# Dicklesworthstone/frankensearch

Hardware: AMD Instinct MI355X
Metric: queries/sec + p50 phase-1 latency, 10M×384 f16 corpus, 1/2/4/8 MI355X (higher is better)
Workload: dtype f16 x f32 -> f32 (every emitted score, in the reference's operation order); candidate filter i8 x i8 -> i32

## Files before the change

frankensearch_amd/csrc/kernels.hpp:

```cpp
#pragma once

#include <hip/hip_runtime.h>
#include <stddef.h>
#include <stdint.h>

namespace fsgpu {

typedef unsigned long long u64;

struct ScanArgs {
    const void* slab;
    const u64* live;
    const u64* allow;
    const float* queries;
    u64* partial;
    uint32_t nrows;
    uint32_t dim;
    uint32_t k;
    uint32_t row_base;
    int32_t hreduce;
    uint32_t row_stride;
};

struct MergeArgs {
// ... 153 lines not shown
                                 hipStream_t stream);
hipError_t launch_prepare_queries_i8(const float* q, uint32_t nq, uint32_t nq_pad, uint32_t dim, void* qi8, float* delta,
                                     hipStream_t stream, int bits = 8);
hipError_t launch_prepare_queries_i8_filter(const float* q, uint32_t nq, uint32_t nq_pad, uint32_t dim, uint32_t q_stride,
                                            const unsigned int* slab_max_bits, const unsigned int* slab_stats, void* qi8,
                                            float* delta, hipStream_t stream, float* unit_out = nullptr, double extra_coeff = 0.0);

constexpr uint32_t kMfmaMaxSlots = 32;
constexpr uint32_t kMfmaSpillCountStride = 16;
constexpr uint32_t kWideSlots = 32;
bool scan_mfma_supported(int dim);
bool scan_wide_supported(int dim, int elem_bytes);
bool scan_wide_group_maxima_supported(int dim, int query_tiles);
int scan_wide_max_query_tiles(int dim, int elem_bytes);
hipError_t launch_scan_wide(const MfmaScanArgs& args, int query_tiles, int grid, hipStream_t stream, int* occupancy);
bool scan_wide_flat_priority();
void note_main_pass_kernel(const char* name);
const char* last_main_pass_kernel();
int scan_mfma_waves_per_block(int shape);
int scan_mfma_rows_per_tile(int shape);
int scan_mfma_query_tiles(int shape);
int scan_mfma_max_slots(int shape);
bool scan_mfma_shape_built(int shape);
int scan_mfma_planner_shape(int requested, int elem_bytes);
hipError_t launch_scan_mfma(const MfmaScanArgs& args, int shape, int grid, hipStream_t stream, int* occupancy);
hipError_t launch_max_row_norm(const void* slab, uint32_t nrows, uint32_t dim, uint32_t row_stride_bytes, unsigned int* out_bits,
                               hipStream_t stream);
hipError_t launch_max_row_norm_f32(const float* rows, uint32_t nrows, uint32_t dim, unsigned int* out_bits, hipStream_t stream);
hipError_t launch_prepare_queries(const float* q, uint32_t nq, uint32_t nq_pad, uint32_t dim, uint32_t q_stride,
                                  const unsigned int* max_norm_bits, void* qh, float* delta, hipStream_t stream);
// ... 322 lines not shown
```

frankensearch_amd/csrc/mfma_wide.hip:

```cpp
#include <atomic>
#include <cstdlib>
#include <string>
#include <vector>
#include <type_traits>

#include "scan_common.hpp"

namespace fsgpu {

using namespace scan_detail;

typedef float f32x4 __attribute__((ext_vector_type(4)));
typedef int i32x4 __attribute__((ext_vector_type(4)));

namespace {

__device__ __forceinline__ void glds16(const void* gsrc, uint32_t lds_dst) {
    unsigned keep;
    asm volatile(
        "s_mov_b32 %0, m0\n\t"
        "s_mov_b32 m0, %2\n\t"
        "s_nop 0\n\t"
        "global_load_lds_dwordx4 %1, off\n\t"
        "s_mov_b32 m0, %0"
// ... 39 lines not shown

__device__ __forceinline__ int ceil_threshold(float t) {
    if (!(t <= 33554432.0f)) return 1 << 25;
    if (t < -33554432.0f) return -(1 << 25);
    return (int)ceilf(t);
}

__device__ __forceinline__ bool wave_any(bool x) { return __ballot(x) != 0; }

template <int N>
__device__ __forceinline__ void wait_vmcnt() {
    static_assert(N >= 0 && N < 64, "vmcnt is a 6-bit field");
    asm volatile("s_waitcnt vmcnt(%0)" ::"n"(N) : "memory");
}

[[maybe_unused]] __device__ __forceinline__ void flag_post(uint32_t lds_addr, int lane) {
    asm volatile("" ::: "memory");
    if (lane == 0) {
        const uint32_t one = 1;
        asm volatile("ds_add_u32 %0, %1" ::"v"(lds_addr), "v"(one) : "memory");
    }
}
[[maybe_unused]] __device__ __forceinline__ void flag_wait(uint32_t lds_addr, uint32_t target) {
    for (;;) {
        uint32_t v;
        asm volatile("ds_read_b32 %0, %1\n\ts_waitcnt lgkmcnt(0)" : "=v"(v) : "v"(lds_addr) : "memory");
        if ((uint32_t)__builtin_amdgcn_readfirstlane(v) >= target) break;
        __builtin_amdgcn_s_sleep(1);
    }
    asm volatile("" ::: "memory");
}

}

constexpr int kOptNegTau = 2, kOptSaddr = 4, kOptSplit = 8, kOptBig = 16, kOptFlags = 32, kOptFlat = 64;

constexpr int wide_level(int h, int H) { return 3 - (h * 4) / H; }

constexpr int wide_chunk_ksteps(int KS, int QT) {
    return KS == 12 ? (QT >= 3 ? 2 : 3) : KS == 6 ? (QT >= 5 ? 1 : 3) : KS == 4 ? (QT >= 7 ? 1 : 2) : (KS >= 2 ? KS / 2 : 1);
}
constexpr bool wide_room(int ROWB, int QT) {
    const int KS = ROWB / 64;
    return QT * KS * 4 + 4 * wide_chunk_ksteps(KS, QT) * 4 + 8 * QT <= 190;
}
constexpr bool wide_split_ok(int ROWB, int EB, int QT, int OPT, int DBG) {
    const int KS = ROWB / 64;
    return (OPT & kOptSplit) != 0 && (OPT & kOptNegTau) != 0 && EB == 1 && wide_room(ROWB, QT) && ROWB < 512 && QT >= 2 && DBG != 1 &&
           QT * KS * 4 + 2 * KS * 4 + 9 * QT <= 200;
}
// ... 48 lines not shown
    r[2] = wi;
    r[3] = (unsigned long long)which | ((unsigned long long)(uintptr_t)p << 8);
    r[4] = sv;
    r[5] = vv;
    r[6] = sv2;
    r[7] = vv2;
}
#endif

template <int ROWB, int EB, int QT, int NSLOT, int OPT, int DBG, int WPBT, int NQB>
__device__ __forceinline__ void scan_wide_body(MfmaScanArgs args, const int q0_wave) {
    using acc_t = std::conditional_t<EB == 2, f32x4, i32x4>;
    constexpr int WPB = WPBT, NT = WPB * 64;
    constexpr int KS = ROWB / 64;
    constexpr bool BIG = wide_big_ok(ROWB, EB, QT, NSLOT, OPT, DBG);
    constexpr bool FLAGS = BIG && (OPT & kOptFlags) != 0;
    constexpr int TR = BIG ? 128 : ROWB >= 512 ? 32 : 64;
    constexpr int RS = TR / 16;
    constexpr int NI = RS * KS;
    constexpr int PW = NI / WPB;
    static_assert(NI % WPB == 0 && PW >= 1, "a tile's DMA instructions divide evenly over the 8 waves");
    static_assert(RS % 2 == 0, "sub-tiles are consumed in pairs");
    constexpr int CK = wide_chunk_ksteps(KS, QT);
    constexpr int NCH = KS / CK;
    constexpr int NC = (RS / 2) * NCH;
    static_assert(KS % CK == 0 && NC % 2 == 0, "an even number of chunks per tile: the register double buffer starts every tile in the same phase");
    static_assert(NSLOT >= 3, "tile n is consumed while n+1 .. n+NSLOT-2 are in flight and n-1's slot is being refilled");
    constexpr bool ROOM = wide_room(ROWB, QT);
    constexpr bool NEGTAU = (OPT & kOptNegTau) != 0 && EB == 1 && ROOM;
    constexpr bool SADDR = (OPT & kOptSaddr) != 0 && ROOM;
    constexpr bool SPLIT = wide_split_ok(ROWB, EB, QT, OPT, DBG);
    constexpr bool LEVEL = SPLIT && (OPT & kOptFlat) == 0;
    constexpr bool GMAX = DBG == 7 && SPLIT && EB == 1;
    constexpr bool SK = DBG >= 16 && DBG < 32;
    constexpr bool SK_NO_DMA = DBG == 2 || (SK && (DBG & 1)), SK_NO_SYNC = SK && (DBG & 2), SK_NO_READS = SK && (DBG & 4), SK_NO_TEST = SK && (DBG & 8);
    constexpr bool AK = DBG >= 32;
    [[maybe_unused]] constexpr bool AK_NO_STORE = AK && (DBG & 1), AK_NO_ATOMIC = AK && (DBG & 2), AK_NO_BODY = AK && (DBG & 4);
    constexpr bool STAMPS = DBG == 8;
    [[maybe_unused]] unsigned long long st_loop = 0, st_bar = 0;
    static_assert(!SPLIT || (NEGTAU && RS >= 4), "the split loop runs on neg-tau accumulators over tiles of two pairs or more");
    constexpr bool NT4 = NEGTAU && !SPLIT && QT * KS * 4 + 4 * CK * 4 + 12 * QT <= 200 && QT * KS * 4 <= 96;
    constexpr int TILE_BYTES = TR * ROWB;
    constexpr int NQ = NQB;
    if (gridDim.y > 1) {
        const uint32_t grp = blockIdx.y;
        args.queries = static_cast<const unsigned char*>(args.queries) + (size_t)grp * NQ * ROWB;
        args.tau += (size_t)grp * NQ;
        args.cand += (size_t)grp * NQ * gridDim.x * args.slots;
        if (args.cand_count) args.cand_count += (size_t)grp * NQ * gridDim.x;
        args.spill += (size_t)grp * NQ * args.spill_cap;
        args.spill_count += (size_t)grp * NQ * kMfmaSpillCountStride;
        args.overflow += (size_t)grp * NQ;
        if (!args.side_by_side) args.reverse ^= grp & 1u;
    }
    extern __shared__ __attribute__((aligned(1024))) unsigned char smem[];
    const uint32_t ring = (uint32_t)(uintptr_t)smem;
    int* lcnt = reinterpret_cast<int*>(smem + (size_t)NSLOT * TILE_BYTES);
    const uint32_t flags = ring + (uint32_t)(NSLOT * TILE_BYTES + NQ * 4);
    const int tid = threadIdx.x, lane = tid & 63;
    const int wave = __builtin_amdgcn_readfirstlane(tid >> 6);
    const int frow = lane & 15, fk = lane >> 4;
    const int slots = (int)args.slots;
    for (int i = tid; i < NQ; i += NT) lcnt[i] = 0;
    if (FLAGS && tid < 8) lcnt[NQ + tid] = 0;
    if (STAMPS && tid < 32) lcnt[NQ + 16 + tid] = 0;

    const int q0 = q0_wave;
    half8 bq[QT][KS];
    float tau[QT];
    int ctau[QT];
    i32x4 ntau4[QT];
    {
        const unsigned char* qbase = static_cast<const unsigned char*>(args.queries);
#pragma unroll
        for (int nt = 0; nt < QT; ++nt) {
            const unsigned char* qp = qbase + (size_t)(q0 + nt * 16 + frow) * ROWB + fk * 16;
#pragma unroll
            for (int ks = 0; ks < KS; ++ks) bq[nt][ks] = *reinterpret_cast<const half8*>(qp + ks * 64);
            tau[nt] = GMAX ? 0.f : args.tau[q0 + nt * 16 + frow];
// ... 265 lines not shown
#endif
        }
        if constexpr (STAMPS) {
            const unsigned long long dt = __builtin_readcyclecounter() - st_in;
            if (lane == 0) {
                unsigned long long* st = reinterpret_cast<unsigned long long*>(lcnt + NQ + 16) + wave * 2;
                atomicAdd(st, dt);
                atomicAdd(st + 1, 1ull);
            }
        }
    };
    auto emit_pair = [&](uint32_t t, int sp, const acc_t (&acc)[2][QT]) {
        if (__builtin_expect(wave_any(any_passes(acc, 0, QT)), 0)) emit_tiles(t, sp, acc, 0, QT, 0);
    };

#ifndef FSGPU_LAB_NO_DCACHE_INV
    if (args.live || args.allow) asm volatile("s_dcache_inv\n\ts_waitcnt lgkmcnt(0)" ::: "memory");
#endif
    __syncthreads();
    Cursor cl{0, blockIdx.x, blockIdx.x};
    Cursor cc = cl;
    auto fetch_part = [&](uint32_t slot, int part) {
        uint32_t t = cl.n < rounds ? cursor_tile(cl) : ntiles;
        t = t < ntiles ? t : ntiles - 1;
        issue_part(t, slot, part);
        if (part == PARTS - 1 && cl.n < rounds) cursor_next(cl);
    };
    auto fetch_next = [&](uint32_t slot) {
#pragma unroll
        for (int part = 0; part < PARTS; ++part) fetch_part(slot, part);
// ... 31 lines not shown
        auto mfma_step = [&](int kk, int nt_lo, int nt_hi) {
#pragma unroll
            for (int nt = nt_lo; nt < nt_hi; ++nt)
#pragma unroll
                for (int h = 0; h < 2; ++h)
                    acc[h][nt] = __builtin_amdgcn_mfma_i32_16x16x64_i8(__builtin_bit_cast(i32x4, f[h][kk]),
                                                                       __builtin_bit_cast(i32x4, bq[nt][kk]), acc[h][nt], 0, 0, 0);
        };
        auto init_acc = [&](int nt_lo, int nt_hi) {
#pragma unroll
            for (int h = 0; h < 2; ++h)
#pragma unroll
                for (int nt = nt_lo; nt < nt_hi; ++nt) acc[h][nt] = i32x4{-ctau[nt], -ctau[nt], -ctau[nt], -ctau[nt]};
        };
        wait_vmcnt<PW*(NSLOT - 2)>();
        if constexpr (FLAGS) {
            flag_post(flags, lane);
            flag_wait(flags, WPB);
        } else {
            __builtin_amdgcn_s_barrier();
            asm volatile("" ::: "memory");
        }
#pragma unroll
        for (int kk = 0; kk < KS; ++kk) read_frag(slot_base(0), 0, kk);
        init_acc(0, QT);
        if constexpr (SK_NO_READS) sk_loop = true;
        uint32_t slot = 0, slot_prev = NSLOT - 1;
        const unsigned char* cur = slot_base(0);
        uint32_t tB = ntiles;
        [[maybe_unused]] int gbest[QT];
        [[maybe_unused]] uint32_t grow[QT];
        if constexpr (GMAX) {
#pragma unroll
            for (int nt = 0; nt < QT; ++nt) {
                gbest[nt] = -0x7fffffff - 1;
                grow[nt] = 0;
            }
        }
        auto gmax_update = [&](uint32_t tt, int sp, int nt_lo, int nt_hi) __attribute__((always_inline)) {
            if constexpr (GMAX) {
                const uint32_t g = tile_row0(tt < ntiles ? tt : 0u) + (uint32_t)sp * 16u;
                if (tt < ntiles && g + 32u <= args.nrows) {
                    if (args.live || args.allow) {
                        u64 mask = ~0ull;
// ... 24 lines not shown
                        for (int nt = nt_lo; nt < nt_hi; ++nt) {
                            const int v = lane_max(acc, nt);
                            const bool better = v > gbest[nt];
                            gbest[nt] = better ? v : gbest[nt];
                            grow[nt] = better ? g : grow[nt];
                        }
                    }
                }
            }
        };
        if constexpr (STAMPS) st_loop = __builtin_readcyclecounter();
        while (cc.n < rounds) {
            const uint32_t slot_next = slot + 1 == NSLOT ? 0 : slot + 1;
            const unsigned char* nxt = slot_base(slot_next);
            const uint32_t t = cursor_tile(cc);
#pragma unroll
            for (int p = 0; p < NP; ++p) {
                constexpr int TK = KS >= 4 ? 2 : 0;
                constexpr int H = 2 * NP;
                const int lv1 = wide_level(2 * p, H), lv2 = wide_level(2 * p + 1, H);
                if (lv1 != wide_level((2 * p + H - 1) % H, H)) set_level(lv1);
                init_acc(0, QA);
                bool anyB = false;
#pragma unroll
                for (int kk = 0; kk < KS; ++kk) {
                    mfma_step(kk, 0, QA);
                    if constexpr (GMAX) {
                        if (kk == TK) gmax_update(tB, ((p + NP - 1) % NP) * 2, QA, QT);
                    } else {
                        if (kk == TK) anyB = sk_any(QA, QT);
                    }
                    if (p == 0 && kk == 0 && !SK_NO_SYNC) {
                        [[maybe_unused]] unsigned long long st_a = 0;
                        if constexpr (STAMPS) st_a = __builtin_readcyclecounter();
                        wait_vmcnt<PW*(NSLOT - 3)>();
                        if constexpr (FLAGS) {
                            flag_post(flags + slot_next * 4, lane);
                        } else {
                            __builtin_amdgcn_s_barrier();
                            asm volatile("" ::: "memory");
                        }
                        if constexpr (STAMPS) st_bar += __builtin_readcyclecounter() - st_a;
                    }
                    {
                        constexpr int IPP = (PARTS + NP - 1) / NP;
                        constexpr int K1 = KS >= 3 ? 2 : KS - 1, K2 = KS >= 5 ? 4 : K1;
                        if constexpr (FLAGS) {
                            if (p == 0 && kk == K1 && cc.n >= 1) flag_wait(flags + 16 + slot_prev * 4, WPB * ((cc.n - 1) / NSLOT + 1));
                        }
                        if (kk == K1 && p * IPP < PARTS) fetch_part(slot_prev, p * IPP);
                        if (IPP > 1 && K2 != K1 && kk == K2 && p * IPP + 1 < PARTS) fetch_part(slot_prev, p * IPP + 1);
                    }
                    __builtin_amdgcn_sched_barrier(0);
                }
                if (__builtin_expect(wave_any(anyB), 0)) emit_tiles(tB, ((p + NP - 1) % NP) * 2, acc, QA, QT, lv1);
                if (lv2 != lv1) set_level(lv2);
                init_acc(QA, QT);
                bool anyA = false;
#pragma unroll
                for (int kk = 0; kk < KS; ++kk) {
                    mfma_step(kk, QA, QT);
                    if constexpr (FLAGS) {
                        if (p + 1 == NP && kk == 0) flag_wait(flags + slot_next * 4, WPB * ((cc.n + 1) / NSLOT + 1));
                    }
                    if (p + 1 < NP) read_frag(cur, p + 1, kk);
                    else read_frag(nxt, 0, kk);
                    if constexpr (GMAX) {
                        if (kk == TK) gmax_update(t, p * 2, 0, QA);
                    } else {
                        if (kk == TK) anyA = sk_any(0, QA);
                    }
                    __builtin_amdgcn_sched_barrier(0);
                }
                if constexpr (FLAGS) {
                    if (p + 2 == NP) flag_post(flags + 16 + slot * 4, lane);
                }
                if (__builtin_expect(wave_any(anyA), 0)) emit_tiles(t, p * 2, acc, 0, QA, lv2);
                tB = t;
            }
            cursor_next(cc);
            slot_prev = slot;
            slot = slot_next;
            cur = nxt;
        }
        if constexpr (GMAX) {
            gmax_update(tB, (NP - 1) * 2, QA, QT);
            wait_vmcnt<0>();
#pragma unroll
            for (int nt = 0; nt < QT; ++nt) {
                const u64 e = gbest[nt] == -0x7fffffff - 1 ? kEmpty : pack((float)gbest[nt], args.row_base + grow[nt] + (uint32_t)fk * 4u);
                args.cand[((size_t)(q0 + nt * 16 + frow) * gridDim.x + blockIdx.x) * 4 + fk] = e;
            }
            __syncthreads();
            return;
        } else {
            if (__builtin_expect(wave_any(any_passes(acc, QA, QT)), 0)) emit_tiles(tB, (NP - 1) * 2, acc, QA, QT, 0);
        }
    } else {
// ... 51 lines not shown
    }
    }
    wait_vmcnt<0>();
    if (fk == 0) {
#pragma unroll
        for (int nt = 0; nt < QT; ++nt) lcnt[q0 + nt * 16 + frow] = (int)((lcount >> (6 * nt)) & 63u);
    }
    __syncthreads();
    if constexpr (STAMPS) {
        if (args.dense && lane == 0) {
            const unsigned long long* st = reinterpret_cast<const unsigned long long*>(lcnt + NQ + 16) + wave * 2;
            unsigned long long* out = reinterpret_cast<unsigned long long*>(args.dense) + ((size_t)(blockIdx.y * gridDim.x + blockIdx.x) * WPB + wave) * 4;
            out[0] = __builtin_readcyclecounter() - st_loop;
            out[1] = st_bar;
            out[2] = st[0];
            out[3] = st[1];
        }
    }
    if (args.cand_count) {
        for (int q = tid; q < NQ; q += NT) {
            const int c = lcnt[q];
            args.cand_count[(size_t)q * gridDim.x + blockIdx.x] = (uint32_t)(c < slots ? c : slots);
        }
        return;
    }
    for (int i = tid; i < NQ * slots; i += NT) {
        const int q = i / slots, j = i - q * slots;
        if (j >= lcnt[q]) args.cand[((size_t)q * gridDim.x + blockIdx.x) * slots + j] = kEmpty;
    }
}

// ... 42 lines not shown
        int blocks = 0;
        if (hipOccupancyMaxActiveBlocksPerMultiprocessor(&blocks, kern, 512, lds) != hipSuccess || blocks < 1) blocks = 1;
        *occupancy = blocks;
        return hipSuccess;
    }
    if (args.slots > kWideSlots) return hipErrorInvalidValue;
    static const std::string name = "scan_wide_kernel<" + std::to_string(ROWB) + ", " + std::to_string(EB) + ", " +
                                    std::to_string(QT) + ", " + std::to_string(NSLOT) + ", " + std::to_string(OPT) + ">";
    if (DBG != 3 && DBG != 7) note_main_pass_kernel(name.c_str());
    hipLaunchKernelGGL(kern, dim3(grid, args.groups ? args.groups : 1), dim3(512), lds, stream, args);
    return hipGetLastError();
}

template <int ROWB, int EB, int QT, int NSLOT, int OPT, int DBG = 0>
hipError_t launch_wide_t(const MfmaScanArgs& args, int grid, hipStream_t stream, int* occupancy) {
    return launch_wide_k<ROWB, EB, QT, NSLOT, wide_split_ok(ROWB, EB, QT, OPT, DBG) ? OPT : (OPT & ~kOptFlat), DBG>(args, grid, stream, occupancy);
}

#ifdef FSGPU_LAB_ASYM
template <int ROWB, int EB, int QTA, int QTB, int NSLOT, int OPT>
hipError_t launch_wide_asym(const MfmaScanArgs& args, int grid, hipStream_t stream) {
    constexpr size_t ring = (size_t)NSLOT * 64 * ROWB;
    const size_t lds = ring + (size_t)64 * (QTA + QTB) * 4 + 64;
    auto kern = scan_wide_asym_kernel<ROWB, EB, QTA, QTB, NSLOT, OPT>;
    static bool attr_done = false;
    if (!attr_done) {
        hipError_t e = hipFuncSetAttribute(reinterpret_cast<const void*>(kern), hipFuncAttributeMaxDynamicSharedMemorySize, (int)lds);
        if (e != hipSuccess) return e;
        attr_done = true;
    }
    if (args.slots > kWideSlots) return hipErrorInvalidValue;
    note_main_pass_kernel("scan_wide_kernel<384, 1, asym>");
    hipLaunchKernelGGL(kern, dim3(grid, args.groups ? args.groups : 1), dim3(512), lds, stream, args);
    return hipGetLastError();
}
#endif

template <int ROWB, int EB, int QT, int NSLOT, int O, int MODE>
hipError_t launch_wide_pick(const MfmaScanArgs& args, int grid, hipStream_t stream, int* occupancy) {
    if constexpr (MODE == 0 && wide_big_ok(ROWB, EB, QT, 3, O, 0)) return launch_wide_t<ROWB, EB, QT, 3, O, 0>(args, grid, stream, occupancy);
    else return launch_wide_t<ROWB, EB, QT, NSLOT, O & ~(kOptBig | kOptFlags), MODE>(args, grid, stream, occupancy);
}

template <int EB, int QT, int MODE, int O>
hipError_t launch_wide_o(const MfmaScanArgs& args, int grid, hipStream_t stream, int* occupancy) {
    if (QT * (int)(args.dim * EB / 64) * 4 > 144) return hipErrorInvalidValue;
    switch (args.dim * EB / 2) {
        case 384: if constexpr (QT <= 3 && MODE != 7) {
#ifdef FSGPU_EXPERIMENTS
            if constexpr (MODE == 0 && EB == 2 && QT == 2) {
                static const int dbg = wide_env("FSGPU_WIDE_DBG");
                if (dbg == 1) return launch_wide_t<768, EB, QT, 6, O, 1>(args, grid, stream, occupancy);
                if (dbg == 2) return launch_wide_t<768, EB, QT, 6, O, 2>(args, grid, stream, occupancy);
            }
#endif
            return launch_wide_t<768, EB, QT, 6, O & ~(kOptBig | kOptFlags), MODE>(args, grid, stream, occupancy);
        } else return hipErrorInvalidValue;
        case 256: if constexpr (QT <= 4 && MODE != 7) return launch_wide_t<512, EB, QT, 8, O & ~kOptFlags, MODE>(args, grid, stream, occupancy);
                  else return hipErrorInvalidValue;
        case 192: if constexpr (EB != 1 || (MODE == 7 && !wide_split_ok(384, 1, QT, O, 7))) return hipErrorInvalidValue; else {
#ifdef FSGPU_EXPERIMENTS
            if constexpr (EB == 1 && QT == 4) {
                static const int opt = wide_env("FSGPU_WIDE_OPT");
                static const int dbg = wide_env("FSGPU_WIDE_DBG");
                if constexpr (MODE == 0) {
                    if (dbg == 1) return launch_wide_t<384, EB, QT, 6, 6, 1>(args, grid, stream, occupancy);
                    if (dbg == 2) return launch_wide_t<384, EB, QT, 6, 6, 2>(args, grid, stream, occupancy);
                    if (dbg == 4) return launch_wide_t<384, EB, QT, 6, 6, 4>(args, grid, stream, occupancy);
                    if (dbg == 5) return launch_wide_t<384, EB, QT, 6, 6, 5>(args, grid, stream, occupancy);
                }
                switch (opt) {
                    case 0: return launch_wide_t<384, EB, QT, 6, 0, MODE>(args, grid, stream, occupancy);
                    case 2: return launch_wide_t<384, EB, QT, 6, 2, MODE>(args, grid, stream, occupancy);
                    case 4: return launch_wide_t<384, EB, QT, 6, 4, MODE>(args, grid, stream, occupancy);
                    case 6: return launch_wide_t<384, EB, QT, 6, 6, MODE>(args, grid, stream, occupancy);
                    case 14: return launch_wide_t<384, EB, QT, 6, 14, MODE>(args, grid, stream, occupancy);
                    case 30:
                        if constexpr (MODE == 0) return launch_wide_t<384, EB, QT, 3, 30, MODE>(args, grid, stream, occupancy);
                        else return launch_wide_t<384, EB, QT, 6, 14, MODE>(args, grid, stream, occupancy);
                    default: break;
                }
                if constexpr (MODE == 0) {
                    if (dbg == 8 && !occupancy) {
                        static unsigned long long* buf = nullptr;
                        constexpr size_t kWords = 2 * 1024 * 8 * 4;
                        if (!buf && hipMalloc(reinterpret_cast<void**>(&buf), kWords * 8) != hipSuccess) return hipErrorOutOfMemory;
                        MfmaScanArgs a2 = args;
                        a2.dense = reinterpret_cast<u64*>(buf);
                        (void)hipMemsetAsync(buf, 0, kWords * 8, stream);
                        const hipError_t e = launch_wide_t<384, EB, QT, 3, O, 8>(a2, grid, stream, nullptr);
                        if (e != hipSuccess) return e;
                        (void)hipStreamSynchronize(stream);
                        const size_t nwaves = (size_t)grid * (args.groups ? args.groups : 1) * 8;
                        std::vector<unsigned long long> h(nwaves * 4);
                        (void)hipMemcpy(h.data(), buf, h.size() * 8, hipMemcpyDeviceToHost);
                        double loop = 0, bar[2] = {0, 0}, slow[2] = {0, 0}, ent[2] = {0, 0}, lp[2] = {0, 0};
                        int hist[10] = {0};
                        for (size_t w = 0; w < nwaves; ++w) {
                            const double L = (double)h[w * 4], B = (double)h[w * 4 + 1], S = (double)h[w * 4 + 2], E = (double)h[w * 4 + 3];
                            if (L <= 0) continue;
                            const int half = (w & 7) >= 4;
                            loop += L;
                            lp[half] += L;
                            bar[half] += B;
                            slow[half] += S;
                            ent[half] += E;
                            int b = (int)(10.0 * B / L);
                            ++hist[b < 0 ? 0 : b > 9 ? 9 : b];
                        }
                        std::fprintf(stderr, "[wide stamps] waves %zu  loop cycles/wave %.0f | at the tile's wait + barrier: waves 0-3 %.1f %%, waves 4-7 %.1f %% | in the append path: "
                                             "%.1f %% / %.1f %% (%.0f / %.0f entries per wave, %.0f cycles each) | waves by barrier share, deciles:",
                                     nwaves, loop / nwaves, 100 * bar[0] / lp[0], 100 * bar[1] / lp[1], 100 * slow[0] / lp[0], 100 * slow[1] / lp[1],
                                     ent[0] / (nwaves / 2), ent[1] / (nwaves / 2), (slow[0] + slow[1]) / std::max(1.0, ent[0] + ent[1]));
                        for (int b = 0; b < 10; ++b) std::fprintf(stderr, " %d", hist[b]);
                        std::fprintf(stderr, "\n");
                        return hipSuccess;
                    }
                    switch (dbg) {
#define FSGPU_SK(D) case D: return launch_wide_t<384, EB, QT, 3, O, D>(args, grid, stream, occupancy);
                        FSGPU_SK(16) FSGPU_SK(17) FSGPU_SK(18) FSGPU_SK(20) FSGPU_SK(24) FSGPU_SK(31) FSGPU_SK(33) FSGPU_SK(35) FSGPU_SK(36)
#undef FSGPU_SK
                        default: break;
                    }
                }
            }
#endif
#ifdef FSGPU_LAB_ASYM
            if constexpr (EB == 1 && QT == 4 && MODE == 0) { if (!occupancy) return launch_wide_asym<384, 1, FSGPU_LAB_ASYM, 8 - FSGPU_LAB_ASYM, 6, O & ~(kOptBig | kOptFlags)>(args, grid, stream); }
#endif
            return launch_wide_pick<384, EB, QT, 6, O, MODE>(args, grid, stream, occupancy);
        }
        case 128: if constexpr (EB != 1 || (MODE == 7 && !wide_split_ok(256, 1, QT, O, 7))) return hipErrorInvalidValue;
                  else return launch_wide_pick<256, EB, QT, 8, O, MODE>(args, grid, stream, occupancy);
        default: return hipErrorInvalidValue;
    }
}

template <int EB, int QT, int MODE = 0>
hipError_t launch_wide_d(const MfmaScanArgs& args, int grid, hipStream_t stream, int* occupancy) {
    if (scan_wide_flat_priority()) return launch_wide_o<EB, QT, MODE, kWideOptDefault | kOptFlat>(args, grid, stream, occupancy);
    return launch_wide_o<EB, QT, MODE, kWideOptDefault>(args, grid, stream, occupancy);
}

}

#ifdef FSGPU_LAB_BITMAP_CHECK
extern "C" int fsgpu_lab_bitmap_debug(unsigned long long* out, int cap_records) {
    unsigned int n = 0;
    if (hipMemcpyFromSymbol(&n, HIP_SYMBOL(g_bm_dbg_n), 4) != hipSuccess) return -1;
    const int take = (int)(n < 64u ? n : 64u) < cap_records ? (int)(n < 64u ? n : 64u) : cap_records;
    if (take > 0 && hipMemcpyFromSymbol(out, HIP_SYMBOL(g_bm_dbg), (size_t)take * 64) != hipSuccess) return -1;
    return (int)n;
}
#endif

bool scan_wide_supported(int dim, int elem_bytes) {
    const int rowb = dim * elem_bytes;
    return rowb == 768 || rowb == 512 || (elem_bytes == 1 && (rowb == 384 || rowb == 256));
}

bool scan_wide_group_maxima_supported(int dim, int query_tiles) {
    return (dim == 384 || dim == 256) && query_tiles >= 2 && query_tiles <= 5 &&
           wide_split_ok(dim, 1, query_tiles, kWideOptDefault, 7);
}

int scan_wide_max_query_tiles(int dim, int elem_bytes) {
    const int per_tile = dim * elem_bytes / 64 * 4;
    const int fit = per_tile > 0 ? 144 / per_tile : 0;
    if (elem_bytes != 1) return fit > 3 ? 3 : fit;
// ... 29 lines not shown
```

frankensearch_amd/csrc/vector_index_batched.cpp:

```cpp
#include "vector_index.hpp"

#include <algorithm>
#include <cmath>
#include <cstdio>
#include <cstdlib>
#include <chrono>
#include <cstring>

#include "../../include/fsgpu.h"
#include "lab_env.hpp"
#include "vector_index_internal.hpp"

namespace fsgpu {

using namespace detail;

bool scan_wide_flat_priority() { return knobs().wide_flat_priority; }

SearchError VectorIndex::search_top_k_batched_device(const float* queries_dev, uint32_t nq, uint32_t query_len,
                                                     uint32_t k, const uint64_t* allow_dev, uint32_t* out_rows_dev,
                                                     float* out_scores_dev, uint32_t* out_counts_dev,
                                                     hipStream_t stream, uint32_t* fallbacks, uint64_t* out_packed_dev) {
    BatchedRequest rq(queries_dev, nq, query_len, k, stream);
    rq.allow_dev = allow_dev;
    rq.out_rows_dev = out_rows_dev;
    rq.out_scores_dev = out_scores_dev;
    rq.out_counts_dev = out_counts_dev;
    rq.out_packed_dev = out_packed_dev;
    BatchedOutcome o;
    const SearchError e = batched_exact(rq, &o);
    if (fallbacks) *fallbacks = o.fallbacks;
    return e;
// ... 937 lines not shown
    constexpr uint32_t KC = BatchedPlan::KC;
    hipStream_t stream = p.rq.stream;
    const uint32_t nq = p.rq.nq, k = p.rq.k, k_eff = p.k_eff;
    if (!already_waited) FSGPU_HIP(hipStreamSynchronize(stream));
    std::vector<uint32_t> fb;
    for (uint32_t i = 0; i < nq; ++i)
        if (p.overflow_all[i] || p.counts_all[i] < k_eff) fb.push_back(i);
    if (knobs().debug_batched) {
        uint32_t big = 0, slot = 0, few = 0, mx = 0;
        for (uint32_t i = 0; i < nq; ++i) {
            if (p.counts_all[i] > (p.big_pool ? 8192u : KC)) ++big;
            else if (p.overflow_all[i]) ++slot;
            if (p.counts_all[i] < k_eff) ++few;
            mx = std::max(mx, p.counts_all[i]);
        }
        std::fprintf(stderr, "[fsgpu batched] nq=%u k=%u fallbacks=%zu  pool_overflow=%u  slot_or_skip=%u  few=%u  max_cand=%u\n", nq, k,
                     fb.size(), big, slot, few, mx);
        for (size_t j = 0; j < fb.size() && j < 4; ++j)
            std::fprintf(stderr, "    query %u: overflow=%u candidates=%u\n", fb[j], p.overflow_all[fb[j]], p.counts_all[fb[j]]);
    }
    uint32_t total_fallbacks = (uint32_t)fb.size();
    if (total_fallbacks && p.i8 && !p.i8f) {
        std::vector<float> qh(dim_), sc(k);
        std::vector<uint32_t> rw(k);
        for (uint32_t i : fb) {
            uint32_t cnt = 0;
            FSGPU_HIP(hipMemcpyAsync(qh.data(), p.rq.queries_dev + (size_t)i * dim_, (size_t)dim_ * 4, hipMemcpyDeviceToHost, stream));
            FSGPU_HIP(hipStreamSynchronize(stream));
            std::fill(rw.begin(), rw.end(), 0xffffffffu);
            FSGPU_TRY(quantized_two_pass(qh.data(), dim_, k, p.rq.int8_mult, p.rq.bits, rw.data(), sc.data(), &cnt,
                                         p.rq.tp_approx ? p.rq.tp_approx + (size_t)i * p.rq.tp_stride : nullptr,
                                         p.rq.tp_exact ? p.rq.tp_exact + (size_t)i * p.rq.tp_stride : nullptr));
// ... 188 lines not shown
```

frankensearch_amd/csrc/vector_index_internal.hpp:

```cpp
#pragma once

#include <algorithm>
#include <cstdint>
#include <cstdlib>
#include <cstring>
#include <string>
#include <utility>

#include "../../include/fsgpu.h"
#include "vector_index.hpp"

namespace fsgpu {
namespace detail {

inline SearchError ok() { return SearchError{}; }

inline SearchError hip_fail(hipError_t e, const char* what) {
    SearchError err;
    err.code = FSGPU_ERR_DEVICE;
    err.detail = std::string(what) + ": " + hipGetErrorString(e);
    return err;
}

inline SearchError make_error(int32_t code, std::string detail) {
// ... 21 lines not shown

inline uint64_t fnv1a(const char* p, size_t n) {
    uint64_t h = 0xcbf29ce484222325ull;
    for (size_t i = 0; i < n; ++i) {
        h ^= (uint8_t)p[i];
        h *= 0x100000001b3ull;
    }
    return h;
}

struct Knobs {
    int grid_blocks = 0, ra = 0, rb = 0, mfma_shape = 0, mfma_shape_i8 = 0, round = 0, i8_per_cu = 0;
    int wide = -1;
    bool wide_sequential = false;
    bool wide_flat_priority = false;
    int filter = 0;
    int slots_b = 0, slots_main = 0;
    int wide_max = 0;
    int i8f_growth = 0;
    bool no_skip_b = false, use_160 = false, debug_batched = false, no_reverse = false, no_wide_b = false, no_anchor = false;
    bool no_big_pool = false, no_heur_b = false, no_group_sample = false;
    bool narrow_i8f = false;
    int rb_pct = 0;
    int heur_rank = 0;
    int wide_min = 0;
    Knobs() {
        auto env = [](const char* name) { return std::getenv(name); };
        if (const char* w = env("FSGPU_WIDE")) wide = std::atoi(w);
        if (const char* l = env("FSGPU_WIDE_LAYOUT")) wide_sequential = std::strcmp(l, "sequential") == 0;
        if (const char* o = env("FSGPU_WIDE_PRIO")) wide_flat_priority = std::strcmp(o, "off") == 0;
        if (const char* f = env("FSGPU_FILTER")) filter = std::strcmp(f, "f16") == 0 ? 1 : std::strcmp(f, "i8") == 0 ? 2 : 0;
        debug_batched = env("FSGPU_DEBUG_BATCHED") != nullptr;
#ifdef FSGPU_EXPERIMENTS
        auto num = [&](const char* name) {
            const char* e = env(name);
            return e ? std::atoi(e) : 0;
        };
        grid_blocks = num("FSGPU_GRID_BLOCKS");
        ra = num("FSGPU_RA");
        rb = num("FSGPU_RB");
        rb_pct = num("FSGPU_RB_PCT");
        round = num("FSGPU_ROUND");
        i8_per_cu = num("FSGPU_I8_PER_CU");
        mfma_shape = num("FSGPU_MFMA_SHAPE");
        mfma_shape_i8 = num("FSGPU_MFMA_SHAPE_I8");
// ... 122 lines not shown
```

Measured before the change: 375,900.

## Replace workgroup barriers with per-slot LDS counters in the wide i8 scan ring

In the BIG wide-scan path, ring slot synchronisation now defaults to per-slot LDS arrival counters instead of s_barrier: a wave posts with a single-lane ds_add, peeks the counter early and only spins if the target has not been reached by the k-step where the slot is needed. Waves no longer lockstep on every tile, so slow waves should not stall the rest. A bounded poll with an overflow fallback and a timeout counter guards against hangs, and an env knob can restore the barrier. This adds LDS traffic and spin-wait risk, and correctness now depends on the counter targets being right.

```diff
diff --git a/frankensearch_amd/csrc/kernels.hpp b/frankensearch_amd/csrc/kernels.hpp
--- a/frankensearch_amd/csrc/kernels.hpp
+++ b/frankensearch_amd/csrc/kernels.hpp
@@ -191,6 +191,8 @@
 bool scan_wide_group_maxima_supported(int dim, int query_tiles);
 int scan_wide_max_query_tiles(int dim, int elem_bytes);
 hipError_t launch_scan_wide(const MfmaScanArgs& args, int query_tiles, int grid, hipStream_t stream, int* occupancy);
+bool scan_wide_barrier_sync();
+uint32_t scan_wide_poll_timeouts();
 bool scan_wide_flat_priority();
 void note_main_pass_kernel(const char* name);
 const char* last_main_pass_kernel();
diff --git a/frankensearch_amd/csrc/mfma_wide.hip b/frankensearch_amd/csrc/mfma_wide.hip
--- a/frankensearch_amd/csrc/mfma_wide.hip
+++ b/frankensearch_amd/csrc/mfma_wide.hip
@@ -77,26 +77,34 @@
     asm volatile("s_waitcnt vmcnt(%0)" ::"n"(N) : "memory");
 }
 
-[[maybe_unused]] __device__ __forceinline__ void flag_post(uint32_t lds_addr, int lane) {
-    asm volatile("" ::: "memory");
-    if (lane == 0) {
-        const uint32_t one = 1;
-        asm volatile("ds_add_u32 %0, %1" ::"v"(lds_addr), "v"(one) : "memory");
-    }
-}
-[[maybe_unused]] __device__ __forceinline__ void flag_wait(uint32_t lds_addr, uint32_t target) {
-    for (;;) {
-        uint32_t v;
-        asm volatile("ds_read_b32 %0, %1\n\ts_waitcnt lgkmcnt(0)" : "=v"(v) : "v"(lds_addr) : "memory");
-        if ((uint32_t)__builtin_amdgcn_readfirstlane(v) >= target) break;
-        __builtin_amdgcn_s_sleep(1);
-    }
-    asm volatile("" ::: "memory");
-}
-
-}
-
-constexpr int kOptNegTau = 2, kOptSaddr = 4, kOptSplit = 8, kOptBig = 16, kOptFlags = 32, kOptFlat = 64;
+__device__ __forceinline__ void slot_post(uint32_t lds_addr) {
+    const uint32_t a = (uint32_t)__builtin_amdgcn_readfirstlane((int)lds_addr);
+    uint64_t keep;
+    uint32_t va, vone;
+    asm volatile(
+        "s_mov_b64 %0, exec\n\t"
+        "s_mov_b64 exec, 1\n\t"
+        "v_mov_b32 %1, %3\n\t"
+        "v_mov_b32 %2, 1\n\t"
+        "ds_add_u32 %1, %2\n\t"
+        "s_mov_b64 exec, %0"
+        : "=&s"(keep), "=&v"(va), "=&v"(vone)
+        : "s"(a)
+        : "memory");
+}
+__device__ __forceinline__ uint32_t slot_peek(const uint32_t* counter) {
+    return __hip_atomic_load(counter, __ATOMIC_RELAXED, __HIP_MEMORY_SCOPE_WORKGROUP);
+}
+__device__ __forceinline__ bool slot_reached(uint32_t seen, uint32_t target) {
+    return (uint32_t)__builtin_amdgcn_readfirstlane((int)seen) >= target;
+}
+constexpr uint32_t kSlotPollBound = 1u << 20;
+constexpr uint32_t kSlotOpen = 0x40000000u;
+__device__ unsigned int g_wide_poll_timeouts;
+
+}
+
+constexpr int kOptNegTau = 2, kOptSaddr = 4, kOptSplit = 8, kOptBig = 16, kOptBarrier = 32, kOptFlat = 64;
 
 constexpr int wide_level(int h, int H) { return 3 - (h * 4) / H; }
 
@@ -175,7 +183,7 @@
     constexpr int WPB = WPBT, NT = WPB * 64;
     constexpr int KS = ROWB / 64;
     constexpr bool BIG = wide_big_ok(ROWB, EB, QT, NSLOT, OPT, DBG);
-    constexpr bool FLAGS = BIG && (OPT & kOptFlags) != 0;
+    constexpr bool SLOTSYNC = BIG && (OPT & kOptBarrier) == 0;
     constexpr int TR = BIG ? 128 : ROWB >= 512 ? 32 : 64;
     constexpr int RS = TR / 16;
     constexpr int NI = RS * KS;
@@ -198,7 +206,7 @@
     constexpr bool AK = DBG >= 32;
     [[maybe_unused]] constexpr bool AK_NO_STORE = AK && (DBG & 1), AK_NO_ATOMIC = AK && (DBG & 2), AK_NO_BODY = AK && (DBG & 4);
     constexpr bool STAMPS = DBG == 8;
-    [[maybe_unused]] unsigned long long st_loop = 0, st_bar = 0;
+    [[maybe_unused]] unsigned long long st_loop = 0, st_bar = 0, st_max = 0;
     static_assert(!SPLIT || (NEGTAU && RS >= 4), "the split loop runs on neg-tau accumulators over tiles of two pairs or more");
     constexpr bool NT4 = NEGTAU && !SPLIT && QT * KS * 4 + 4 * CK * 4 + 12 * QT <= 200 && QT * KS * 4 <= 96;
     constexpr int TILE_BYTES = TR * ROWB;
@@ -218,12 +226,13 @@
     const uint32_t ring = (uint32_t)(uintptr_t)smem;
     int* lcnt = reinterpret_cast<int*>(smem + (size_t)NSLOT * TILE_BYTES);
     const uint32_t flags = ring + (uint32_t)(NSLOT * TILE_BYTES + NQ * 4);
+    uint32_t* const sync = reinterpret_cast<uint32_t*>(lcnt + NQ);
     const int tid = threadIdx.x, lane = tid & 63;
     const int wave = __builtin_amdgcn_readfirstlane(tid >> 6);
     const int frow = lane & 15, fk = lane >> 4;
     const int slots = (int)args.slots;
     for (int i = tid; i < NQ; i += NT) lcnt[i] = 0;
-    if (FLAGS && tid < 8) lcnt[NQ + tid] = 0;
+    if (SLOTSYNC && tid < 8) sync[tid] = 0;
     if (STAMPS && tid < 32) lcnt[NQ + 16 + tid] = 0;
 
     const int q0 = q0_wave;
@@ -519,6 +528,28 @@
         if (__builtin_expect(wave_any(any_passes(acc, 0, QT)), 0)) emit_tiles(t, sp, acc, 0, QT, 0);
     };
 
+    [[maybe_unused]] auto slot_wait_slow = [&](uint32_t idx, uint32_t target) {
+        [[maybe_unused]] unsigned long long st_a = 0;
+        if constexpr (STAMPS) st_a = __builtin_readcyclecounter();
+        for (uint32_t polls = 0; !slot_reached(slot_peek(sync + idx), target);) {
+            if (__builtin_expect(++polls > kSlotPollBound, 0)) {
+                uint32_t lane_v = threadIdx.x;
+                asm volatile("" : "+v"(lane_v));
+                lane_v &= 63u;
+                for (uint32_t q = lane_v; q < (uint32_t)NQ; q += 64) args.overflow[q] = 1;
+                if (lane_v == 0) atomicAdd(&g_wide_poll_timeouts, 1u);
+                if (lane_v < 8) __hip_atomic_store(sync + lane_v, kSlotOpen, __ATOMIC_RELAXED, __HIP_MEMORY_SCOPE_WORKGROUP);
+                break;
+            }
+            __builtin_amdgcn_s_sleep(1);
+        }
+        if constexpr (STAMPS) {
+            const unsigned long long dt = __builtin_readcyclecounter() - st_a;
+            st_bar += dt;
+            st_max = dt > st_max ? dt : st_max;
+        }
+    };
+
 #ifndef FSGPU_LAB_NO_DCACHE_INV
     if (args.live || args.allow) asm volatile("s_dcache_inv\n\ts_waitcnt lgkmcnt(0)" ::: "memory");
 #endif
@@ -580,9 +611,10 @@
                 for (int nt = nt_lo; nt < nt_hi; ++nt) acc[h][nt] = i32x4{-ctau[nt], -ctau[nt], -ctau[nt], -ctau[nt]};
         };
         wait_vmcnt<PW*(NSLOT - 2)>();
-        if constexpr (FLAGS) {
-            flag_post(flags, lane);
-            flag_wait(flags, WPB);
+        if constexpr (SLOTSYNC) {
+            slot_post(flags);
+            if (!slot_reached(slot_peek(sync), WPB)) slot_wait_slow(0, WPB);
+            asm volatile("" ::: "memory");
         } else {
             __builtin_amdgcn_s_barrier();
             asm volatile("" ::: "memory");
@@ -594,6 +626,7 @@
         uint32_t slot = 0, slot_prev = NSLOT - 1;
         const unsigned char* cur = slot_base(0);
         uint32_t tB = ntiles;
+        [[maybe_unused]] uint32_t sync_cur = WPB;
         [[maybe_unused]] int gbest[QT];
         [[maybe_unused]] uint32_t grow[QT];
         if constexpr (GMAX) {
@@ -648,12 +681,20 @@
             const uint32_t slot_next = slot + 1 == NSLOT ? 0 : slot + 1;
             const unsigned char* nxt = slot_base(slot_next);
             const uint32_t t = cursor_tile(cc);
+            [[maybe_unused]] const uint32_t sync_next = sync_cur + (slot_next == 0 ? WPB : 0);
+            [[maybe_unused]] const uint32_t sync_prev = cc.n >= 1 ? sync_cur - (slot == 0 ? WPB : 0) : 0;
+            [[maybe_unused]] uint32_t seen_freed = 0, seen_landed = 0;
 #pragma unroll
             for (int p = 0; p < NP; ++p) {
                 constexpr int TK = KS >= 4 ? 2 : 0;
                 constexpr int H = 2 * NP;
+#ifdef FSGPU_LAB_LEVEL_PARITY
+                const int lv1 = wide_level(((int)(cc.n & 1u) * NP + p) * 2, 2 * H), lv2 = lv1;
+                if (LEVEL && p % (NP / 2) == 0) set_level(lv1);
+#else
                 const int lv1 = wide_level(2 * p, H), lv2 = wide_level(2 * p + 1, H);
                 if (lv1 != wide_level((2 * p + H - 1) % H, H)) set_level(lv1);
+#endif
                 init_acc(0, QA);
                 bool anyB = false;
 #pragma unroll
@@ -668,22 +709,39 @@
                         [[maybe_unused]] unsigned long long st_a = 0;
                         if constexpr (STAMPS) st_a = __builtin_readcyclecounter();
                         wait_vmcnt<PW*(NSLOT - 3)>();
-                        if constexpr (FLAGS) {
-                            flag_post(flags + slot_next * 4, lane);
+                        if constexpr (SLOTSYNC) {
+                            slot_post(flags + slot_next * 4);
+                            seen_freed = slot_peek(sync + 4 + slot_prev);
                         } else {
                             __builtin_amdgcn_s_barrier();
                             asm volatile("" ::: "memory");
                         }
-                        if constexpr (STAMPS) st_bar += __builtin_readcyclecounter() - st_a;
+                        if constexpr (STAMPS) {
+                            const unsigned long long dt = __builtin_readcyclecounter() - st_a;
+                            st_bar += dt;
+                            st_max = dt > st_max ? dt : st_max;
+                        }
                     }
                     {
                         constexpr int IPP = (PARTS + NP - 1) / NP;
                         constexpr int K1 = KS >= 3 ? 2 : KS - 1, K2 = KS >= 5 ? 4 : K1;
-                        if constexpr (FLAGS) {
-                            if (p == 0 && kk == K1 && cc.n >= 1) flag_wait(flags + 16 + slot_prev * 4, WPB * ((cc.n - 1) / NSLOT + 1));
+                        if constexpr (SLOTSYNC) {
+                            static_assert(K1 >= 1, "the counter is read at k-step 0 and needed at k-step K1");
+                            if (p == 0 && kk == K1) {
+                                if (__builtin_expect(!slot_reached(seen_freed, sync_prev), 0)) slot_wait_slow(4 + slot_prev, sync_prev);
+                                asm volatile("" ::: "memory");
+                            }
                         }
                         if (kk == K1 && p * IPP < PARTS) fetch_part(slot_prev, p * IPP);
                         if (IPP > 1 && K2 != K1 && kk == K2 && p * IPP + 1 < PARTS) fetch_part(slot_prev, p * IPP + 1);
+                    }
+                    if constexpr (SLOTSYNC) {
+                        constexpr int KP = KS >= 3 ? KS - 3 : 0;
+                        if (p + 1 == NP && kk == KP) seen_landed = slot_peek(sync + slot_next);
+                        if (p + 1 == NP && kk == KS - 1) {
+                            if (__builtin_expect(!slot_reached(seen_landed, sync_next), 0)) slot_wait_slow(slot_next, sync_next);
+                            asm volatile("" ::: "memory");
+                        }
                     }
                     __builtin_amdgcn_sched_barrier(0);
                 }
@@ -694,9 +752,6 @@
 #pragma unroll
                 for (int kk = 0; kk < KS; ++kk) {
                     mfma_step(kk, QA, QT);
-                    if constexpr (FLAGS) {
-                        if (p + 1 == NP && kk == 0) flag_wait(flags + slot_next * 4, WPB * ((cc.n + 1) / NSLOT + 1));
-                    }
                     if (p + 1 < NP) read_frag(cur, p + 1, kk);
                     else read_frag(nxt, 0, kk);
                     if constexpr (GMAX) {
@@ -706,8 +761,8 @@
                     }
                     __builtin_amdgcn_sched_barrier(0);
                 }
-                if constexpr (FLAGS) {
-                    if (p + 2 == NP) flag_post(flags + 16 + slot * 4, lane);
+                if constexpr (SLOTSYNC) {
+                    if (p + 2 == NP) slot_post(flags + 16 + slot * 4);
                 }
                 if (__builtin_expect(wave_any(anyA), 0)) emit_tiles(t, p * 2, acc, 0, QA, lv2);
                 tB = t;
@@ -716,6 +771,7 @@
             slot_prev = slot;
             slot = slot_next;
             cur = nxt;
+            if constexpr (SLOTSYNC) sync_cur = sync_next;
         }
         if constexpr (GMAX) {
             gmax_update(tB, (NP - 1) * 2, QA, QT);
@@ -797,7 +853,7 @@
             out[0] = __builtin_readcyclecounter() - st_loop;
             out[1] = st_bar;
             out[2] = st[0];
-            out[3] = st[1];
+            out[3] = st[1] | ((st_max < 0xffffffffull ? st_max : 0xffffffffull) << 32);
         }
     }
     if (args.cand_count) {
@@ -870,7 +926,9 @@
 
 template <int ROWB, int EB, int QT, int NSLOT, int OPT, int DBG = 0>
 hipError_t launch_wide_t(const MfmaScanArgs& args, int grid, hipStream_t stream, int* occupancy) {
-    return launch_wide_k<ROWB, EB, QT, NSLOT, wide_split_ok(ROWB, EB, QT, OPT, DBG) ? OPT : (OPT & ~kOptFlat), DBG>(args, grid, stream, occupancy);
+    constexpr int O1 = wide_split_ok(ROWB, EB, QT, OPT, DBG) ? OPT : (OPT & ~kOptFlat);
+    constexpr int O2 = wide_big_ok(ROWB, EB, QT, NSLOT, OPT, DBG) ? O1 : (O1 & ~kOptBarrier);
+    return launch_wide_k<ROWB, EB, QT, NSLOT, O2, DBG>(args, grid, stream, occupancy);
 }
 
 #ifdef FSGPU_LAB_ASYM
@@ -895,7 +953,7 @@
 template <int ROWB, int EB, int QT, int NSLOT, int O, int MODE>
 hipError_t launch_wide_pick(const MfmaScanArgs& args, int grid, hipStream_t stream, int* occupancy) {
     if constexpr (MODE == 0 && wide_big_ok(ROWB, EB, QT, 3, O, 0)) return launch_wide_t<ROWB, EB, QT, 3, O, 0>(args, grid, stream, occupancy);
-    else return launch_wide_t<ROWB, EB, QT, NSLOT, O & ~(kOptBig | kOptFlags), MODE>(args, grid, stream, occupancy);
+    else return launch_wide_t<ROWB, EB, QT, NSLOT, O & ~kOptBig, MODE>(args, grid, stream, occupancy);
 }
 
 template <int EB, int QT, int MODE, int O>
@@ -910,9 +968,9 @@
                 if (dbg == 2) return launch_wide_t<768, EB, QT, 6, O, 2>(args, grid, stream, occupancy);
             }
 #endif
-            return launch_wide_t<768, EB, QT, 6, O & ~(kOptBig | kOptFlags), MODE>(args, grid, stream, occupancy);
+            return launch_wide_t<768, EB, QT, 6, O & ~kOptBig, MODE>(args, grid, stream, occupancy);
         } else return hipErrorInvalidValue;
-        case 256: if constexpr (QT <= 4 && MODE != 7) return launch_wide_t<512, EB, QT, 8, O & ~kOptFlags, MODE>(args, grid, stream, occupancy);
+        case 256: if constexpr (QT <= 4 && MODE != 7) return launch_wide_t<512, EB, QT, 8, O, MODE>(args, grid, stream, occupancy);
                   else return hipErrorInvalidValue;
         case 192: if constexpr (EB != 1 || (MODE == 7 && !wide_split_ok(384, 1, QT, O, 7))) return hipErrorInvalidValue; else {
 #ifdef FSGPU_EXPERIMENTS
@@ -934,6 +992,9 @@
                     case 30:
                         if constexpr (MODE == 0) return launch_wide_t<384, EB, QT, 3, 30, MODE>(args, grid, stream, occupancy);
                         else return launch_wide_t<384, EB, QT, 6, 14, MODE>(args, grid, stream, occupancy);
+                    case 62:
+                        if constexpr (MODE == 0) return launch_wide_t<384, EB, QT, 3, 62, MODE>(args, grid, stream, occupancy);
+                        else return launch_wide_t<384, EB, QT, 6, 14, MODE>(args, grid, stream, occupancy);
                     default: break;
                 }
                 if constexpr (MODE == 0) {
@@ -952,8 +1013,10 @@
                         (void)hipMemcpy(h.data(), buf, h.size() * 8, hipMemcpyDeviceToHost);
                         double loop = 0, bar[2] = {0, 0}, slow[2] = {0, 0}, ent[2] = {0, 0}, lp[2] = {0, 0};
                         int hist[10] = {0};
+                        unsigned long long longest = 0;
                         for (size_t w = 0; w < nwaves; ++w) {
-                            const double L = (double)h[w * 4], B = (double)h[w * 4 + 1], S = (double)h[w * 4 + 2], E = (double)h[w * 4 + 3];
+                            const double L = (double)h[w * 4], B = (double)h[w * 4 + 1], S = (double)h[w * 4 + 2], E = (double)(h[w * 4 + 3] & 0xffffffffull);
+                            longest = std::max(longest, h[w * 4 + 3] >> 32);
                             if (L <= 0) continue;
                             const int half = (w & 7) >= 4;
                             loop += L;
@@ -964,10 +1027,10 @@
                             int b = (int)(10.0 * B / L);
                             ++hist[b < 0 ? 0 : b > 9 ? 9 : b];
                         }
-                        std::fprintf(stderr, "[wide stamps] waves %zu  loop cycles/wave %.0f | at the tile's wait + barrier: waves 0-3 %.1f %%, waves 4-7 %.1f %% | in the append path: "
-                                             "%.1f %% / %.1f %% (%.0f / %.0f entries per wave, %.0f cycles each) | waves by barrier share, deciles:",
+                        std::fprintf(stderr, "[wide stamps] waves %zu  loop cycles/wave %.0f | at the tile's DMA wait + barrier / slot waits: waves 0-3 %.1f %%, waves 4-7 %.1f %% | in the append path: "
+                                             "%.1f %% / %.1f %% (%.0f / %.0f entries per wave, %.0f cycles each) | longest single wait %llu cycles | waves by wait share, deciles:",
                                      nwaves, loop / nwaves, 100 * bar[0] / lp[0], 100 * bar[1] / lp[1], 100 * slow[0] / lp[0], 100 * slow[1] / lp[1],
-                                     ent[0] / (nwaves / 2), ent[1] / (nwaves / 2), (slow[0] + slow[1]) / std::max(1.0, ent[0] + ent[1]));
+                                     ent[0] / (nwaves / 2), ent[1] / (nwaves / 2), (slow[0] + slow[1]) / std::max(1.0, ent[0] + ent[1]), longest);
                         for (int b = 0; b < 10; ++b) std::fprintf(stderr, " %d", hist[b]);
                         std::fprintf(stderr, "\n");
                         return hipSuccess;
@@ -982,7 +1045,7 @@
             }
 #endif
 #ifdef FSGPU_LAB_ASYM
-            if constexpr (EB == 1 && QT == 4 && MODE == 0) { if (!occupancy) return launch_wide_asym<384, 1, FSGPU_LAB_ASYM, 8 - FSGPU_LAB_ASYM, 6, O & ~(kOptBig | kOptFlags)>(args, grid, stream); }
+            if constexpr (EB == 1 && QT == 4 && MODE == 0) { if (!occupancy) return launch_wide_asym<384, 1, FSGPU_LAB_ASYM, 8 - FSGPU_LAB_ASYM, 6, O & ~kOptBig>(args, grid, stream); }
 #endif
             return launch_wide_pick<384, EB, QT, 6, O, MODE>(args, grid, stream, occupancy);
         }
@@ -992,10 +1055,17 @@
     }
 }
 
+template <int EB, int QT, int MODE, int O>
+hipError_t launch_wide_s(const MfmaScanArgs& args, int grid, hipStream_t stream, int* occupancy) {
+    if constexpr (MODE == 0) {
+        if (scan_wide_barrier_sync()) return launch_wide_o<EB, QT, MODE, O | kOptBarrier>(args, grid, stream, occupancy);
+    }
+    return launch_wide_o<EB, QT, MODE, O>(args, grid, stream, occupancy);
+}
 template <int EB, int QT, int MODE = 0>
 hipError_t launch_wide_d(const MfmaScanArgs& args, int grid, hipStream_t stream, int* occupancy) {
-    if (scan_wide_flat_priority()) return launch_wide_o<EB, QT, MODE, kWideOptDefault | kOptFlat>(args, grid, stream, occupancy);
-    return launch_wide_o<EB, QT, MODE, kWideOptDefault>(args, grid, stream, occupancy);
+    if (scan_wide_flat_priority()) return launch_wide_s<EB, QT, MODE, kWideOptDefault | kOptFlat>(args, grid, stream, occupancy);
+    return launch_wide_s<EB, QT, MODE, kWideOptDefault>(args, grid, stream, occupancy);
 }
 
 }
@@ -1009,6 +1079,12 @@
     return (int)n;
 }
 #endif
+
+uint32_t scan_wide_poll_timeouts() {
+    unsigned int n = 0;
+    if (hipMemcpyFromSymbol(&n, HIP_SYMBOL(g_wide_poll_timeouts), sizeof n) != hipSuccess) return ~0u;
+    return n;
+}
 
 bool scan_wide_supported(int dim, int elem_bytes) {
     const int rowb = dim * elem_bytes;
diff --git a/frankensearch_amd/csrc/vector_index_batched.cpp b/frankensearch_amd/csrc/vector_index_batched.cpp
--- a/frankensearch_amd/csrc/vector_index_batched.cpp
+++ b/frankensearch_amd/csrc/vector_index_batched.cpp
@@ -16,6 +16,7 @@
 using namespace detail;
 
 bool scan_wide_flat_priority() { return knobs().wide_flat_priority; }
+bool scan_wide_barrier_sync() { return knobs().wide_barrier_sync; }
 
 SearchError VectorIndex::search_top_k_batched_device(const float* queries_dev, uint32_t nq, uint32_t query_len,
                                                      uint32_t k, const uint64_t* allow_dev, uint32_t* out_rows_dev,
@@ -983,8 +984,8 @@
             if (p.counts_all[i] < k_eff) ++few;
             mx = std::max(mx, p.counts_all[i]);
         }
-        std::fprintf(stderr, "[fsgpu batched] nq=%u k=%u fallbacks=%zu  pool_overflow=%u  slot_or_skip=%u  few=%u  max_cand=%u\n", nq, k,
-                     fb.size(), big, slot, few, mx);
+        std::fprintf(stderr, "[fsgpu batched] nq=%u k=%u fallbacks=%zu  pool_overflow=%u  slot_or_skip=%u  few=%u  max_cand=%u  slot_wait_timeouts=%u\n", nq, k,
+                     fb.size(), big, slot, few, mx, scan_wide_poll_timeouts());
         for (size_t j = 0; j < fb.size() && j < 4; ++j)
             std::fprintf(stderr, "    query %u: overflow=%u candidates=%u\n", fb[j], p.overflow_all[fb[j]], p.counts_all[fb[j]]);
     }
diff --git a/frankensearch_amd/csrc/vector_index_internal.hpp b/frankensearch_amd/csrc/vector_index_internal.hpp
--- a/frankensearch_amd/csrc/vector_index_internal.hpp
+++ b/frankensearch_amd/csrc/vector_index_internal.hpp
@@ -59,6 +59,7 @@
     int wide = -1;
     bool wide_sequential = false;
     bool wide_flat_priority = false;
+    bool wide_barrier_sync = false;
     int filter = 0;
     int slots_b = 0, slots_main = 0;
     int wide_max = 0;
@@ -74,6 +75,7 @@
         if (const char* w = env("FSGPU_WIDE")) wide = std::atoi(w);
         if (const char* l = env("FSGPU_WIDE_LAYOUT")) wide_sequential = std::strcmp(l, "sequential") == 0;
         if (const char* o = env("FSGPU_WIDE_PRIO")) wide_flat_priority = std::strcmp(o, "off") == 0;
+        if (const char* y = env("FSGPU_WIDE_SYNC")) wide_barrier_sync = std::strcmp(y, "barrier") == 0;
         if (const char* f = env("FSGPU_FILTER")) filter = std::strcmp(f, "f16") == 0 ? 1 : std::strcmp(f, "i8") == 0 ? 2 : 0;
         debug_batched = env("FSGPU_DEBUG_BATCHED") != nullptr;
 #ifdef FSGPU_EXPERIMENTS
```

Measured after the change: 383,100, median of 6. +1.9%, better.
